# muzishen/IMAGHarmony

Hardware: AMD Instinct MI355X
Metric: 1024^2 SDXL images/sec (30 DDIM steps, PNS N seeds) (higher is better)
Workload: dtype bf16

## Files before the change

### imagharmony_amd/csrc/api.hip

```cpp
#include <stdarg.h>
#include <stdio.h>
#include <string.h>

#include <vector>

#include "../../include/imh.h"
#include "../../include/imh_adapter.h"
#include "../../include/imh_regions.h"
#include "imh_common.h"
#include "imh_kernels.h"

namespace imh {

static thread_local char g_err[512] = "";

void set_error(const char* fmt, ...) {
    va_list ap;
    va_start(ap, fmt);
    vsnprintf(g_err, sizeof(g_err), fmt, ap);
    va_end(ap);
}

int experimental_refused(const char* what) {
    set_error("%s is compiled only with -DIMH_EXPERIMENTAL (IMH_EXPERIMENTAL=1 python -m imagharmony_amd.build): measured, not selected by any "
// ... 275 lines not shown
    p.mean[0] = a->mean0; p.mean[1] = a->mean1; p.mean[2] = a->mean2; p.std[0] = a->std0; p.std[1] = a->std1; p.std[2] = a->std2;
    p.ncols = p.ntx = p.nty = p.RC = 0;
    return clip_preprocess_launch(p, a->dtype, s);
}

static int do_control_add(const imh_control_add_args* a, hipStream_t s) {
    const char* who = "imh_control_add";
    if (!a || !a->x || !a->r || !a->y) { set_error("%s: null pointer argument", who); return IMH_ERR_ARG; }
    if (((uintptr_t)a->x | (uintptr_t)a->r | (uintptr_t)a->y) & 15) { set_error("%s: x, r and y must be 16-byte aligned", who); return IMH_ERR_ARG; }
    if (((uintptr_t)a->partial | (uintptr_t)a->tab | (uintptr_t)a->step) & 3) { set_error("%s: partial, tab and step must be 4-byte aligned", who); return IMH_ERR_ARG; }
    if ((a->tab == nullptr) != (a->step == nullptr)) { set_error("%s: tab and step come together", who); return IMH_ERR_ARG; }
    if (a->B <= 0 || a->HW <= 0 || a->C <= 0 || a->Br <= 0) { set_error("%s: B=%d Br=%d HW=%d C=%d must be positive", who, a->B, a->Br, a->HW, a->C); return IMH_ERR_SHAPE; }
    const size_t yb = (size_t)a->B * a->HW * a->C * 2, rb = (size_t)a->Br * a->HW * a->C * 2;
    const uintptr_t y0 = (uintptr_t)a->y, x0 = (uintptr_t)a->x, r0 = (uintptr_t)a->r;
    if ((y0 < x0 + yb && x0 < y0 + yb) || (y0 < r0 + rb && r0 < y0 + yb)) { set_error("%s: y must not overlap x or r (no in-place form)", who); return IMH_ERR_ARG; }
    ControlAddParams p;
    p.x = a->x; p.r = a->r; p.y = a->y; p.partial = a->partial; p.tab = a->tab; p.step = a->step; p.scale = a->scale;
    p.B = a->B; p.Br = a->Br; p.HW = a->HW; p.C = a->C; p.sub = a->sub;
    return control_add_launch(p, a->dtype, s);
}

static int do_adapter_op(const imh_adapter_args* a, hipStream_t s) {
    const char* who = "imh_adapter_op";
    if (!a || !a->x || !a->y) { set_error("%s: null pointer argument", who); return IMH_ERR_ARG; }
    if (a->mode != IMH_ADAPTER_UNSHUFFLE && a->mode != IMH_ADAPTER_RELU && a->mode != IMH_ADAPTER_AVGPOOL2) {
        set_error("%s: unknown mode %d", who, a->mode); return IMH_ERR_ARG;
    }
    if (((uintptr_t)a->y & 15) || ((uintptr_t)a->x & (a->mode == IMH_ADAPTER_UNSHUFFLE ? 3 : 15))) {
        set_error("%s: y (and x, unshuffle: to 4 bytes) must be 16-byte aligned", who); return IMH_ERR_ARG;
    }
    if (a->dtype != IMH_DT_BF16 && a->dtype != IMH_DT_F16) { set_error("%s: unknown dtype %d", who, a->dtype); return IMH_ERR_DTYPE; }
    const long long lim = 0x7fffffffLL;
    long long xe, ye;
    if (a->mode == IMH_ADAPTER_RELU) {
        if (a->n <= 0 || a->n > lim) { set_error("%s: relu over n=%lld elements (0 < n < 2^31)", who, (long long)a->n); return IMH_ERR_SHAPE; }
        xe = ye = a->n;
    } else {
        if (a->N <= 0 || a->C <= 0 || a->H <= 0 || a->W <= 0) { set_error("%s: N=%d C=%d H=%d W=%d must be positive", who, a->N, a->C, a->H, a->W); return IMH_ERR_SHAPE; }
        xe = (long long)a->N * a->C;
        if (xe > lim || (xe *= a->H) > lim || (xe *= a->W) > lim) { set_error("%s: N=%d C=%d H=%d W=%d: an operand of 2^31 elements or more", who, a->N, a->C, a->H, a->W); return IMH_ERR_SHAPE; }
        if (a->mode == IMH_ADAPTER_UNSHUFFLE) {
            if (a->f < 1 || a->H % a->f || a->W % a->f) { set_error("%s: unshuffle of %d x %d by f=%d (f >= 1 divides both sides)", who, a->H, a->W, a->f); return IMH_ERR_SHAPE; }
            const long long K = (long long)a->C * a->f * a->f;
            if (a->Cp <= 0 || a->Cp % 8 || a->Cp < K) { set_error("%s: Cp=%d must be a multiple of 8 and at least C f^2 = %lld", who, a->Cp, K); return IMH_ERR_SHAPE; }
            ye = (long long)a->N * (a->H / a->f) * (a->W / a->f);
            if (ye > lim || (ye *= a->Cp) > lim) { set_error("%s: Cp=%d: an operand of 2^31 elements or more", who, a->Cp); return IMH_ERR_SHAPE; }
        } else {
            if (a->C % 8) { set_error("%s: avgpool2 over C=%d channels (a multiple of 8)", who, a->C); return IMH_ERR_SHAPE; }
            ye = (long long)a->N * ((a->H + 1) / 2) * ((a->W + 1) / 2) * a->C;
        }
    }
    const uintptr_t x0 = (uintptr_t)a->x, y0 = (uintptr_t)a->y;
    const size_t xb = (size_t)xe * (a->mode == IMH_ADAPTER_UNSHUFFLE ? 4 : 2), yb = (size_t)ye * 2;
    if (y0 < x0 + xb && x0 < y0 + yb && !(a->mode == IMH_ADAPTER_RELU && x0 == y0)) {
        set_error("%s: y must not overlap x (relu: except y == x)", who); return IMH_ERR_ARG;
    }
    AdapterParams p;
    p.x = a->x; p.y = a->y; p.n = a->n; p.mode = a->mode; p.N = a->N; p.C = a->C; p.H = a->H; p.W = a->W; p.f = a->f; p.Cp = a->Cp;
    return adapter_launch(p, a->dtype, s);
}

}

using namespace imh;

struct imh_op {
    int kind;
    int ew_op;
    int tag;
    union {
        imh_gemm_args gemm;
        imh_attn_args attn;
        imh_norm_args norm;
        imh_ew_args ew;
        imh_small_attn_args sattn;
        imh_gemm_args gemm2[2];
        imh_xattn_args xattn;
        imh_enc_attn_args eattn;
        imh_seeded_args seeded;
        imh_randn_args randn;
        imh_clip_preprocess_args clip;
        imh_control_add_args cadd;
        imh_xattn_regions_args xregions;
    } u;
};

struct imh_plan {
    std::vector<imh_op> ops;
    hipGraph_t graph = nullptr;
    hipGraphExec_t exec = nullptr;
};

struct op_entry {
    int kind;
    size_t size;
    int (*run)(const imh_op&, hipStream_t);
};
static const op_entry g_ops[] = {
    {IMH_OP_GEMM, sizeof(imh_gemm_args), [](const imh_op& o, hipStream_t s) { return do_gemm(&o.u.gemm, s); }},
    {IMH_OP_ATTN, sizeof(imh_attn_args), [](const imh_op& o, hipStream_t s) { return do_attn(&o.u.attn, s); }},
    {IMH_OP_GROUPNORM, sizeof(imh_norm_args), [](const imh_op& o, hipStream_t s) { return do_groupnorm(&o.u.norm, s); }},
    {IMH_OP_LAYERNORM, sizeof(imh_norm_args), [](const imh_op& o, hipStream_t s) { return do_layernorm(&o.u.norm, s); }},
    {IMH_OP_EW, sizeof(imh_ew_args), [](const imh_op& o, hipStream_t s) { return do_ew(o.ew_op, &o.u.ew, s); }},
    {IMH_OP_ATTN_SMALL, sizeof(imh_small_attn_args), [](const imh_op& o, hipStream_t s) { return do_attn_small(&o.u.sattn, s); }},
    {IMH_OP_GEMM_DUAL, 2 * sizeof(imh_gemm_args), [](const imh_op& o, hipStream_t s) { return do_gemm_dual(&o.u.gemm2[0], &o.u.gemm2[1], s); }},
    {IMH_OP_XATTN, sizeof(imh_xattn_args), [](const imh_op& o, hipStream_t s) { return do_xattn(&o.u.xattn, s); }},
    {IMH_OP_ATTN_ENC, sizeof(imh_enc_attn_args), [](const imh_op& o, hipStream_t s) { return do_attn_enc(&o.u.eattn, s); }},
    {IMH_OP_ATTN_ENC_CAUSAL, sizeof(imh_enc_attn_args), [](const imh_op& o, hipStream_t s) { return do_attn_enc(&o.u.eattn, s, 1); }},
    {IMH_OP_STEP_SEEDED, sizeof(imh_seeded_args), [](const imh_op& o, hipStream_t s) { return do_step_seeded(&o.u.seeded, s); }},
    {IMH_OP_RANDN_SEEDED, sizeof(imh_randn_args), [](const imh_op& o, hipStream_t s) { return do_randn_seeded(&o.u.randn, s); }},
    {IMH_OP_CLIP_PREPROCESS, sizeof(imh_clip_preprocess_args), [](const imh_op& o, hipStream_t s) { return do_clip_preprocess(&o.u.clip, s); }},
    {IMH_OP_CONTROL_ADD, sizeof(imh_control_add_args), [](const imh_op& o, hipStream_t s) { return do_control_add(&o.u.cadd, s); }},
    {IMH_OP_XATTN_REGIONS, sizeof(imh_xattn_regions_args), [](const imh_op& o, hipStream_t s) { return do_xattn_regions(&o.u.xregions, s); }},
};

static const op_entry* find_op(int kind) {
    for (const op_entry& e : g_ops)
        if (e.kind == kind) return &e;
    return nullptr;
}

static int run_op(const imh_op& o, hipStream_t s) {
    const op_entry* e = find_op(o.kind);
    if (!e) { set_error("plan: unknown op kind %d", o.kind); return IMH_ERR_ARG; }
    return e->run(o, s);
}

static void drop_graph(imh_plan* p) {
    if (p->exec) { hipGraphExecDestroy(p->exec); p->exec = nullptr; }
    if (p->graph) { hipGraphDestroy(p->graph); p->graph = nullptr; }
}

extern "C" {

int imh_abi_version(void) { return IMH_ABI_VERSION; }
int imh_debug_set(int key, int value) {
    if (key == 0) { g_attn_force_nw = value; return IMH_OK; }
    if (key == 1) {
#ifdef IMH_EXPERIMENTAL
        return 1;
#else
        return 0;
#endif
    }
    if (key == 2) { g_xcd_mode = value; return IMH_OK; }
    if (key == 3) { g_xattn_mode = value; return IMH_OK; }
    if (key == 4) { g_attn_mode = value; return IMH_OK; }
    if (key == 5) { g_halo_mode = value; return IMH_OK; }
    if (key == 7) { g_w16_pf = value; return IMH_OK; }
    if (key == 9) { g_w16_form = value; return IMH_OK; }
    if (key == 10) { g_f32_exact = value; return IMH_OK; }
    if (key == 11) { if (value >= 0) g_up_phase = value; return g_up_phase; }
    if (key == 6) { g_ws_early = value; return IMH_OK; }
    set_error("debug_set: unknown key %d", key);
    return IMH_ERR_ARG;
}
const char* imh_last_error(void) { return g_err; }

int imh_gemm(const imh_gemm_args* a, void* stream) { return do_gemm(a, (hipStream_t)stream); }
int imh_gemm_dual(const imh_gemm_args* a, const imh_gemm_args* b, void* stream) { return do_gemm_dual(a, b, (hipStream_t)stream); }
int imh_gemm_pick_config(int M, int N, int K, int* bm, int* bn, int* splits) {
    if (!bm || !bn || !splits) { set_error("pick_config: null output"); return IMH_ERR_ARG; }
    gemm_pick_config(M, N, K, bm, bn, splits);
    return IMH_OK;
}
size_t imh_gemm_workspace_bytes(int M, int N, int splits) { return gemm_workspace_bytes(M, N, splits); }
int imh_gemm_stats_slot_width(int bm, int bn) { return gemm_stats_slot_width(bm, bn); }
int imh_gemm_gn_block_rows(int bm, int bn) { return gemm_gn_block_rows(bm, bn); }
int imh_conv_halo_lds_bytes(int bm, int bn, int Cin, int gn) { return conv_halo_lds_bytes(bm, bn, Cin, gn); }

int imh_gemm_check(const imh_gemm_args* a) {
    static thread_local std::vector<hipStream_t> streams;
    int dev = -1;
    if (hipGetDevice(&dev) != hipSuccess || dev < 0) { (void)hipGetLastError(); set_error("gemm_check: no current device"); return IMH_ERR_LAUNCH; }
    if ((size_t)dev >= streams.size()) streams.resize(dev + 1, nullptr);
    hipStream_t& cs = streams[dev];
    if (!cs && hipStreamCreateWithFlags(&cs, hipStreamNonBlocking) != hipSuccess) {
        cs = nullptr; (void)hipGetLastError();
        set_error("gemm_check: no stream to validate on"); return IMH_ERR_LAUNCH;
    }
    hipError_t e = hipStreamBeginCapture(cs, hipStreamCaptureModeThreadLocal);
    if (e != hipSuccess) { (void)hipGetLastError(); set_error("gemm_check: begin: %s", hipGetErrorString(e)); return IMH_ERR_LAUNCH; }
    const int rc = do_gemm(a, cs);
    hipGraph_t g = nullptr;
    e = hipStreamEndCapture(cs, &g);
    if (g) hipGraphDestroy(g);
    if (rc != IMH_OK) { (void)hipGetLastError(); return rc; }
    if (e != hipSuccess) { (void)hipGetLastError(); set_error("gemm_check: end: %s", hipGetErrorString(e)); return IMH_ERR_LAUNCH; }
    return IMH_OK;
}

int imh_attention(const imh_attn_args* a, void* stream) { return do_attn(a, (hipStream_t)stream); }

int imh_cross_attention(const imh_xattn_args* a, void* stream) { return do_xattn(a, (hipStream_t)stream); }

int imh_cross_attention_regions(const imh_xattn_regions_args* a, void* stream) { return do_xattn_regions(a, (hipStream_t)stream); }

int imh_attention_small(const imh_small_attn_args* a, void* stream) { return do_attn_small(a, (hipStream_t)stream); }

int imh_attention_enc(const imh_enc_attn_args* a, void* stream) { return do_attn_enc(a, (hipStream_t)stream); }
int imh_attention_enc_causal(const imh_enc_attn_args* a, void* stream) { return do_attn_enc(a, (hipStream_t)stream, 1); }

int imh_groupnorm(const imh_norm_args* a, void* stream) { return do_groupnorm(a, (hipStream_t)stream); }
size_t imh_groupnorm_workspace_bytes(int B, int HW, int C, int groups) { return groupnorm_workspace_bytes(B, HW, C, groups); }
int imh_groupnorm_stats_blocks(int HW, int C) { return groupnorm_stats_blocks(HW, C); }
int imh_groupnorm_stats_sub(int C, int groups) { return groups > 0 && C % groups == 0 ? groupnorm_stats_sub(C, groups) : 0; }
int imh_layernorm(const imh_norm_args* a, void* stream) { return do_layernorm(a, (hipStream_t)stream); }

int imh_elementwise(int op, const imh_ew_args* a, void* stream) { return do_ew(op, a, (hipStream_t)stream); }

int imh_step_seeded(const imh_seeded_args* a, void* stream) { return do_step_seeded(a, (hipStream_t)stream); }
int imh_randn_seeded(const imh_randn_args* a, void* stream) { return do_randn_seeded(a, (hipStream_t)stream); }
int imh_clip_preprocess(const imh_clip_preprocess_args* a, void* stream) { return do_clip_preprocess(a, (hipStream_t)stream); }
int imh_control_add(const imh_control_add_args* a, void* stream) { return do_control_add(a, (hipStream_t)stream); }
int imh_adapter_op(const imh_adapter_args* a, void* stream) { return do_adapter_op(a, (hipStream_t)stream); }
int imh_randn_seeded_host(const imh_randn_args* a) {
    RandnParams p;
    const int rc = to_randn(a, "imh_randn_seeded_host", &p);
    return rc != IMH_OK ? rc : randn_seeded_host(p);
}

int imh_f32(int op, const imh_f32_args* a, void* stream) {
    if (!a) { set_error("imh_f32: null args"); return IMH_ERR_ARG; }
    F32Params p;
    p.X = a->X; p.W = a->W; p.Y = a->Y; p.bias = a->bias; p.residual = a->residual; p.gamma = a->gamma; p.beta = a->beta; p.ws = a->ws;
    p.M = a->M; p.N = a->N; p.K = a->K; p.ldx = a->ldx; p.ldw = a->ldw; p.ldy = a->ldy; p.ldr = a->ldr;
    p.conv = a->conv; p.H = a->H; p.Wd = a->Wd; p.Cin = a->Cin; p.Ho = a->Ho; p.Wo = a->Wo; p.up = a->up;
    p.B = a->B; p.HW = a->HW; p.C = a->C; p.groups = a->groups; p.nblk = a->nblk; p.silu = a->silu;
    p.eps = a->eps; p.scale = a->scale;
    if (a->pad != 0 && a->pad != 1) { set_error("imh_f32: pad must be 0 or 1"); return IMH_ERR_ARG; }
    p.stride = a->stride > 0 ? a->stride : 1; p.pad_lo = a->pad == 1 ? 0 : 1;
    p.add_a = a->add_a; p.add_b = a->add_b;
    return f32_launch(op, p, (hipStream_t)stream);
}

imh_plan* imh_plan_create(void) { return new (std::nothrow) imh_plan(); }
void imh_plan_destroy(imh_plan* p) {
    if (!p) return;
    drop_graph(p);
    delete p;
}
int imh_plan_add(imh_plan* p, int kind, const void* args, int ew_op, int tag) {
    if (!p || !args) { set_error("plan_add: null argument"); return IMH_ERR_ARG; }
    const op_entry* e = find_op(kind);
    if (!e) { set_error("plan_add: unknown kind %d", kind); return IMH_ERR_ARG; }
    imh_op o;
    memset(&o, 0, sizeof(o));
    o.kind = kind; o.ew_op = ew_op; o.tag = tag;
    memcpy(&o.u, args, e->size);
    p->ops.push_back(o);
    drop_graph(p);
    return (int)p->ops.size() - 1;
}
int imh_plan_size(const imh_plan* p) { return p ? (int)p->ops.size() : 0; }
int imh_plan_update(imh_plan* p, int index, const void* args) {
    if (!p || !args || index < 0 || index >= (int)p->ops.size()) { set_error("plan_update: bad index"); return IMH_ERR_ARG; }
    memcpy(&p->ops[index].u, args, find_op(p->ops[index].kind)->size);
    drop_graph(p);
    return IMH_OK;
}
int imh_plan_run_range(imh_plan* p, int first, int last, void* stream) {
    if (!p || first < 0 || last > (int)p->ops.size() || first > last) { set_error("plan_run: bad range"); return IMH_ERR_ARG; }
    for (int i = first; i < last; ++i) {
        int rc = run_op(p->ops[i], (hipStream_t)stream);
        if (rc != IMH_OK) return rc;
    }
    return IMH_OK;
}
int imh_plan_run(imh_plan* p, void* stream) { return imh_plan_run_range(p, 0, p ? (int)p->ops.size() : 0, stream); }

int imh_plan_capture(imh_plan* p, void* stream) {
    if (!p) { set_error("plan_capture: null plan"); return IMH_ERR_ARG; }
    drop_graph(p);
    hipStream_t s = (hipStream_t)stream;
    hipError_t e = hipStreamBeginCapture(s, hipStreamCaptureModeThreadLocal);
    if (e != hipSuccess) { set_error("plan_capture: begin: %s", hipGetErrorString(e)); return IMH_ERR_LAUNCH; }
    int rc = imh_plan_run(p, stream);
    e = hipStreamEndCapture(s, &p->graph);
    if (rc != IMH_OK) { drop_graph(p); return rc; }
    if (e != hipSuccess) { set_error("plan_capture: end: %s", hipGetErrorString(e)); drop_graph(p); return IMH_ERR_LAUNCH; }
    e = hipGraphInstantiate(&p->exec, p->graph, nullptr, nullptr, 0);
    if (e != hipSuccess) { set_error("plan_capture: instantiate: %s", hipGetErrorString(e)); drop_graph(p); return IMH_ERR_LAUNCH; }
    return IMH_OK;
}
int imh_plan_replay(imh_plan* p, void* stream) {
    if (!p || !p->exec) { set_error("plan_replay: plan not captured"); return IMH_ERR_ARG; }
    hipError_t e = hipGraphLaunch(p->exec, (hipStream_t)stream);
    if (e != hipSuccess) { set_error("plan_replay: %s", hipGetErrorString(e)); return IMH_ERR_LAUNCH; }
    return IMH_OK;
}
int imh_plan_time_ops(imh_plan* p, void* stream, float* ms, int n) {
    if (!p || !ms || n < (int)p->ops.size()) { set_error("plan_time_ops: bad arguments"); return IMH_ERR_ARG; }
    hipStream_t s = (hipStream_t)stream;
    const int cnt = (int)p->ops.size();
    std::vector<hipEvent_t> ev(cnt + 1);
    for (auto& e : ev) hipEventCreate(&e);
    int rc = IMH_OK;
    hipEventRecord(ev[0], s);
    for (int i = 0; i < cnt && rc == IMH_OK; ++i) {
        rc = run_op(p->ops[i], s);
        hipEventRecord(ev[i + 1], s);
    }
    hipStreamSynchronize(s);
    if (rc == IMH_OK)
        for (int i = 0; i < cnt; ++i) hipEventElapsedTime(&ms[i], ev[i], ev[i + 1]);
    for (auto& e : ev) hipEventDestroy(e);
// ... 11 lines not shown
```

### imagharmony_amd/csrc/elementwise.hip

```cpp
#include <algorithm>

#include "imh_common.h"
#include "imh_kernels.h"
#include "imh_philox.h"

namespace imh {

enum : int { EW_TIMESTEP = 0, EW_SILU = 1, EW_CONCAT = 2, EW_CONV_IN = 3, EW_CFG_STEP = 4, EW_CAST_F32 = 5,
             EW_ADD = 6, EW_STEP_SET = 7, EW_CFG_RESCALE = 8, EW_SOFTMAX = 9, EW_ROW_STATS = 10, EW_STEP_ROW = 11, EW_GATHER_ROWS = 12,
             EW_CFG_MSTEP = 13 };

template <typename T>
__global__ void timestep_kernel(const EwParams p) {
    const int dim = p.i0, half = dim >> 1;
    const long long total = p.n * half;
    for (long long i = (long long)blockIdx.x * blockDim.x + threadIdx.x; i < total; i += (long long)gridDim.x * blockDim.x) {
        const int v = (int)(i / half), j = (int)(i % half);
        const float t = p.step ? ((const float*)p.a)[*p.step] : ((const float*)p.a)[v];
        const float f = expf(-9.210340371976184f * (float)j / (float)half);
        const float a = t * f;
        T* y = (T*)p.y + (size_t)v * dim;
        y[j] = from_f32<T>(cosf(a));
        y[half + j] = from_f32<T>(sinf(a));
    }
}

template <typename T>
__global__ void silu_kernel(const EwParams p) {
    typedef typename Vec<T>::v8 v8;
    const long long nv = p.n >> 3;
    for (long long i = (long long)blockIdx.x * blockDim.x + threadIdx.x; i < nv; i += (long long)gridDim.x * blockDim.x) {
        v8 v = ((const v8*)p.a)[i], o;
#pragma unroll
        for (int e = 0; e < 8; ++e) o[e] = from_f32<T>(silu_f(to_f32(v[e])));
        ((v8*)p.y)[i] = o;
    }
}

template <typename T>
__global__ void add_kernel(const EwParams p) {
    typedef typename Vec<T>::v8 v8;
    const long long nv = p.n >> 3;
    for (long long i = (long long)blockIdx.x * blockDim.x + threadIdx.x; i < nv; i += (long long)gridDim.x * blockDim.x) {
        v8 u = ((const v8*)p.a)[i], v = ((const v8*)p.b)[i], o;
#pragma unroll
        for (int e = 0; e < 8; ++e) o[e] = from_f32<T>(to_f32(u[e]) + to_f32(v[e]));
        ((v8*)p.y)[i] = o;
    }
}

template <typename T>
__global__ void concat_kernel(const EwParams p) {
    typedef typename Vec<T>::v8 v8;
    const int c1 = p.i0 >> 3, c2 = p.i1 >> 3, ct = c1 + c2;
    const long long total = p.n * ct;
    for (long long i = (long long)blockIdx.x * blockDim.x + threadIdx.x; i < total; i += (long long)gridDim.x * blockDim.x) {
        const long long pix = i / ct;
        const int c = (int)(i - pix * ct);
        v8 v = c < c1 ? ((const v8*)p.a)[pix * c1 + c] : ((const v8*)p.b)[pix * c2 + (c - c1)];
        ((v8*)p.y)[i] = v;
    }
}

template <typename T, int CIN>
__global__ __launch_bounds__(CIN > 4 ? 512 : 256) void conv_in_kernel(const EwParams p) {
    typedef typename Vec<T>::v8 v8;
    constexpr int KT = CIN * 9;
    extern __shared__ float wl[];
    const int S = p.i0, H = p.i1, W = p.i2, C0 = p.i3, Bout = p.i4;
    const T* w = (const T*)p.w;
    for (int co = threadIdx.x; co < C0; co += blockDim.x) {
#pragma unroll
        for (int k = 0; k < KT; ++k) wl[k * C0 + co] = to_f32(w[co * KT + k]);
    }
    for (int i = threadIdx.x; i < C0; i += blockDim.x) wl[KT * C0 + i] = p.bias ? to_f32(((const T*)p.bias)[i]) : 0.f;
    __syncthreads();
    const int cg = C0 >> 3;
    const float in_scale = p.tab ? p.tab[*p.step] : p.f0;
    const long long total = (long long)Bout * H * W * 8;
    const float* lat = (const float*)p.a;
    for (long long i = (long long)blockIdx.x * blockDim.x + threadIdx.x; i < total; i += (long long)gridDim.x * blockDim.x) {
        const int l8 = (int)(i & 7);
        const long long pix = i >> 3;
        const int x = (int)(pix % W);
        const int y = (int)((pix / W) % H);
        const int b = (int)(pix / ((long long)W * H));
        const float* src = lat + (size_t)(b % S) * 4 * H * W;
        float tap[KT];
#pragma unroll
        for (int ci = 0; ci < 4; ++ci)
#pragma unroll
            for (int ky = 0; ky < 3; ++ky)
#pragma unroll
                for (int kx = 0; kx < 3; ++kx) {
                    const int iy = y + ky - 1, ix = x + kx - 1;
                    const bool in = iy >= 0 && iy < H && ix >= 0 && ix < W;
                    const float v = in ? src[((size_t)ci * H + iy) * W + ix] * in_scale : 0.f;
                    tap[ci * 9 + ky * 3 + kx] = to_f32(from_f32<T>(v));
                }
        if constexpr (CIN > 4) {
            const float* src2 = p.x2 + (size_t)(b % S) * (CIN - 4) * H * W;
#pragma unroll
            for (int ci = 4; ci < CIN; ++ci)
#pragma unroll
                for (int ky = 0; ky < 3; ++ky)
#pragma unroll
                    for (int kx = 0; kx < 3; ++kx) {
                        const int iy = y + ky - 1, ix = x + kx - 1;
                        const bool in = iy >= 0 && iy < H && ix >= 0 && ix < W;
                        const float v = in ? src2[((size_t)(ci - 4) * H + iy) * W + ix] : 0.f;
                        tap[ci * 9 + ky * 3 + kx] = to_f32(from_f32<T>(v));
                    }
        }
        for (int c8 = l8; c8 < cg; c8 += 8) {
            float acc[8];
#pragma unroll
            for (int e = 0; e < 8; ++e) acc[e] = wl[KT * C0 + c8 * 8 + e];
#pragma unroll
            for (int k = 0; k < KT; ++k) {
                const float* wr = wl + k * C0 + c8 * 8;
#pragma unroll
                for (int e = 0; e < 8; ++e) acc[e] += tap[k] * wr[e];
            }
            v8 o;
#pragma unroll
            for (int e = 0; e < 8; ++e) o[e] = from_f32<T>(acc[e]);
            ((v8*)p.y)[pix * cg + c8] = o;
        }
    }
}

template <typename T, bool BLEND>
__global__ void cfg_step_kernel(const EwParams p) {
    const int S = p.i0, HW = p.i1;
    const long long total = (long long)S * HW * 4;
    const T* np_ = (const T*)p.a;
    float* lat = (float*)p.y;
    const float cx = p.tab ? p.tab[*p.step * 2] : p.f0;
    const float ce = p.tab ? p.tab[*p.step * 2 + 1] : p.f1;
    float ba = 0.f, bb = 0.f;
    if constexpr (BLEND) { ba = p.blend_tab[*p.step * 2]; bb = p.blend_tab[*p.step * 2 + 1]; }
    for (long long i = (long long)blockIdx.x * blockDim.x + threadIdx.x; i < total; i += (long long)gridDim.x * blockDim.x) {
        const int pix = (int)(i % HW);
        const int ch = (int)((i / HW) % 4);
        const int s = (int)(i / ((long long)HW * 4));
        if (!BLEND || np_) {
            float eps;
            if (p.i3) {
                const float u = to_f32(np_[((size_t)s * HW + pix) * 4 + ch]);
                const float c = to_f32(np_[((size_t)(S + s) * HW + pix) * 4 + ch]);
                eps = u + p.f2 * (c - u);
            } else {
                eps = to_f32(np_[((size_t)s * HW + pix) * 4 + ch]);
            }
            if (p.w) eps *= ((const float*)p.w)[s];
            if (p.b) ((float*)p.b)[i] = eps;
            lat[i] = cx * lat[i] + ce * eps;
        }
        if constexpr (BLEND) {
            const float m = p.mask[(size_t)(s % p.i4) * HW + pix];
            const float pv = ba * p.x2[i] + bb * p.noise[i];
            lat[i] = (1.0f - m) * pv + m * lat[i];
        }
    }
}

template <typename T, bool BLEND, bool SEEDED = false>
__global__ void cfg_mstep_kernel(const EwParams p) {
    const int S = p.i0, HW = p.i1;
    const long long total = (long long)S * HW * 4;
    const T* np_ = (const T*)p.a;
    float* lat = (float*)p.y;
    float* hist = (float*)p.b;
    const int row = *p.step;
    const float* c = p.tab + (size_t)row * 6;
    const float cx = c[0], ce = c[1], ch = c[2], cn = c[3], hx = c[4], he = c[5];
    const float* z = p.bias ? (const float*)p.bias + (size_t)row * (size_t)total : nullptr;
    float ba = 0.f, bb = 0.f;
    if constexpr (BLEND) { ba = p.blend_tab[row * 2]; bb = p.blend_tab[row * 2 + 1]; }
    if constexpr (SEEDED) {
        const bool gen = cn != 0.f;
        const long long quads = (long long)S * HW;
        for (long long q = (long long)blockIdx.x * blockDim.x + threadIdx.x; q < quads; q += (long long)gridDim.x * blockDim.x) {
            const int s = (int)(q / HW);
            PhiloxNormals zn = {{0.f, 0.f, 0.f, 0.f}};
            if (gen) zn = seeded_normals(p.seeds + (size_t)s * 4, (uint32_t)(q - (long long)s * HW), (uint32_t)row, p.noise_stream);
#pragma unroll
            for (int k = 0; k < 4; ++k) {
                const long long i = q * 4 + k;
                const int pix = (int)(i % HW);
                const int chn = (int)((i / HW) % 4);
                float eps;
                if (p.i3) {
                    const float u = to_f32(np_[((size_t)s * HW + pix) * 4 + chn]);
                    const float cnd = to_f32(np_[((size_t)(S + s) * HW + pix) * 4 + chn]);
                    eps = u + p.f2 * (cnd - u);
                } else {
                    eps = to_f32(np_[((size_t)s * HW + pix) * 4 + chn]);
                }
                if (p.w) eps *= ((const float*)p.w)[s];
                const float x = lat[i];
                float y = cx * x + ce * eps;
                if (hist) {
                    y += ch * hist[i];
                    hist[i] = hx * x + he * eps;
                }
                if (gen) y += cn * zn.z[k];
                if constexpr (BLEND) {
                    const float m = p.mask[(size_t)(s % p.i4) * HW + pix];
                    const float pv = ba * p.x2[i] + bb * p.noise[i];
                    y = (1.0f - m) * pv + m * y;
                }
                lat[i] = y;
            }
        }
        return;
    }
    for (long long i = (long long)blockIdx.x * blockDim.x + threadIdx.x; i < total; i += (long long)gridDim.x * blockDim.x) {
        const int pix = (int)(i % HW);
        const int chn = (int)((i / HW) % 4);
        const int s = (int)(i / ((long long)HW * 4));
        float eps;
        if (p.i3) {
            const float u = to_f32(np_[((size_t)s * HW + pix) * 4 + chn]);
            const float cnd = to_f32(np_[((size_t)(S + s) * HW + pix) * 4 + chn]);
            eps = u + p.f2 * (cnd - u);
        } else {
            eps = to_f32(np_[((size_t)s * HW + pix) * 4 + chn]);
        }
        if (p.w) eps *= ((const float*)p.w)[s];
        const float x = lat[i];
        float y = cx * x + ce * eps;
        if (hist) {
            y += ch * hist[i];
            hist[i] = hx * x + he * eps;
        }
        if (z) y += cn * z[i];
        if constexpr (BLEND) {
            const float m = p.mask[(size_t)(s % p.i4) * HW + pix];
            const float pv = ba * p.x2[i] + bb * p.noise[i];
            y = (1.0f - m) * pv + m * y;
        }
        lat[i] = y;
    }
}

__global__ void randn_seeded_kernel(const RandnParams p) {
    const int HW = p.HW;
    const uint32_t row = p.step ? (uint32_t)*p.step : p.row;
    const long long quads = (long long)p.S * HW;
    for (long long q = (long long)blockIdx.x * blockDim.x + threadIdx.x; q < quads; q += (long long)gridDim.x * blockDim.x) {
        const int s = (int)(q / HW);
        const uint32_t qs = p.quad0 + (uint32_t)(q - (long long)s * HW);
        if (p.raw) {
            const PhiloxWords w = seeded_words(p.seeds + (size_t)s * 4, qs, row, p.noise_stream);
            uint32_t* y = (uint32_t*)p.y + q * 4;
#pragma unroll
            for (int k = 0; k < 4; ++k) y[k] = w.w[k];
        } else {
            const PhiloxNormals n = seeded_normals(p.seeds + (size_t)s * 4, qs, row, p.noise_stream);
            float* y = (float*)p.y + q * 4;
#pragma unroll
            for (int k = 0; k < 4; ++k) y[k] = n.z[k];
        }
    }
}

template <typename T>
__global__ __launch_bounds__(256) void cfg_rescale_kernel(const EwParams p) {
    __shared__ double red[4][256];
    const int S = p.i0, HW = p.i1, s = blockIdx.x;
    const long long n = (long long)HW * 4;
    const T* u = (const T*)p.a + (size_t)s * n;
    const T* c = (const T*)p.a + (size_t)(S + s) * n;
    double st = 0, st2 = 0, sc = 0, sc2 = 0;
    for (long long i = threadIdx.x; i < n; i += 256) {
        const float uu = to_f32(u[i]), cc = to_f32(c[i]);
        const float g = uu + p.f2 * (cc - uu);
        st += cc; st2 += (double)cc * cc; sc += g; sc2 += (double)g * g;
    }
    red[0][threadIdx.x] = st; red[1][threadIdx.x] = st2; red[2][threadIdx.x] = sc; red[3][threadIdx.x] = sc2;
// ... 1 lines not shown
    for (int o = 128; o > 0; o >>= 1) {
        if ((int)threadIdx.x < o)
#pragma unroll
            for (int k = 0; k < 4; ++k) red[k][threadIdx.x] += red[k][threadIdx.x + o];
        __syncthreads();
    }
    if (threadIdx.x == 0) {
        const double N = (double)n;
        const double vt = (red[1][0] - red[0][0] * red[0][0] / N) / (N - 1.0);
        const double vc = (red[3][0] - red[2][0] * red[2][0] / N) / (N - 1.0);
        const double ratio = sqrt(fmax(vt, 0.0)) / sqrt(fmax(vc, 1e-300));
        ((float*)p.y)[s] = (float)(p.f3 * ratio + (1.0 - p.f3));
    }
}

template <typename T>
__global__ __launch_bounds__(256) void softmax_rows_kernel(const EwParams p) {
    __shared__ float red[4];
    const int cols = p.i1, lane = threadIdx.x & 63, wave = threadIdx.x >> 6;
    const float* a = (const float*)p.a + (size_t)blockIdx.x * p.i2;
    T* y = (T*)p.y + (size_t)blockIdx.x * p.i3;
    const float c = p.f0 * 1.4426950408889634f;
    float m = -3.0e38f;
    for (int i = threadIdx.x * 4; i < cols; i += 1024) {
        const f32x4 v = *(const f32x4*)(a + i);
        m = fmaxf(fmaxf(m, fmaxf(v[0], v[1])), fmaxf(v[2], v[3]));
    }
    m = wave_max(m);
    if (lane == 0) red[wave] = m;
    __syncthreads();
    m = fmaxf(fmaxf(red[0], red[1]), fmaxf(red[2], red[3]));
    __syncthreads();
    const float mc = m * c;
    float s = 0.f;
    for (int i = threadIdx.x * 4; i < cols; i += 1024) {
        const f32x4 v = *(const f32x4*)(a + i);
#pragma unroll
        for (int e = 0; e < 4; ++e) s += __builtin_amdgcn_exp2f(v[e] * c - mc);
    }
    s = wave_sum(s);
    if (lane == 0) red[wave] = s;
    __syncthreads();
    const float inv = 1.0f / ((red[0] + red[1]) + (red[2] + red[3]));
    for (int i = threadIdx.x * 4; i < cols; i += 1024) {
        const f32x4 v = *(const f32x4*)(a + i);
        typename Vec<T>::v4 o;
#pragma unroll
        for (int e = 0; e < 4; ++e) o[e] = from_f32<T>(__builtin_amdgcn_exp2f(v[e] * c - mc) * inv);
        *(typename Vec<T>::v4*)(y + i) = o;
    }
}

template <typename T>
__global__ void step_row_kernel(const EwParams p) {
    typedef typename Vec<T>::v8 v8;
    const long long nv = p.n >> 3;
    const v8* src = (const v8*)p.a + (long long)(*p.step) * nv;
    for (long long i = (long long)blockIdx.x * blockDim.x + threadIdx.x; i < nv; i += (long long)gridDim.x * blockDim.x) ((v8*)p.y)[i] = src[i];
}

template <typename T>
__global__ void gather_rows_kernel(const EwParams p) {
    typedef typename Vec<T>::v8 v8;
    const int cv = p.i0 >> 3;
    const long long total = p.n * cv;
    const int* idx = (const int*)p.b;
    for (long long i = (long long)blockIdx.x * blockDim.x + threadIdx.x; i < total; i += (long long)gridDim.x * blockDim.x) {
        const long long r = i / cv;
        const int c = (int)(i - r * cv) * 8;
        const int src = idx[r];
        if ((unsigned)src >= (unsigned)p.i5) continue;
        v8 v = *(const v8*)((const T*)p.a + (size_t)src * p.i1 + c);
        if (p.w) {
            const v8 u = *(const v8*)((const T*)p.w + (size_t)(r % p.i3) * p.i4 + c);
#pragma unroll
            for (int e = 0; e < 8; ++e) v[e] = from_f32<T>(to_f32(v[e]) + to_f32(u[e]));
        }
        *(v8*)((T*)p.y + (size_t)r * p.i2 + c) = v;
    }
}

__global__ void step_set_kernel(int* step, int value, int set) {
    if (threadIdx.x == 0 && blockIdx.x == 0) *step = set ? value : *step + 1;
}

template <typename T>
__global__ void cast_f32_kernel(const EwParams p) {
    for (long long i = (long long)blockIdx.x * blockDim.x + threadIdx.x; i < p.n; i += (long long)gridDim.x * blockDim.x)
        ((float*)p.y)[i] = to_f32(((const T*)p.a)[i]);
}

static inline int grid_for(long long work, int threads) {
    long long g = (work + threads - 1) / threads;
    return (int)(g < 1 ? 1 : (g > 4096 ? 4096 : g));
}

template <typename T>
__global__ __launch_bounds__(256) void row_stats_kernel(const EwParams p) {
    const int lane = threadIdx.x & 63;
    const long long row = (long long)blockIdx.x * 4 + (threadIdx.x >> 6);
    if (row >= p.n) return;
    const T* x = (const T*)p.a + row * p.i1;
    const int C = p.i0;
    float s = 0.f;
    for (int c = lane * 8; c < C; c += 512) {
        const typename Vec<T>::v8 t = *(const typename Vec<T>::v8*)(x + c);
#pragma unroll
        for (int e = 0; e < 8; ++e) s += to_f32(t[e]);
    }
    s = wave_sum(s);
    const float mean = s / (float)C;
    float m2 = 0.f;
    for (int c = lane * 8; c < C; c += 512) {
        const typename Vec<T>::v8 t = *(const typename Vec<T>::v8*)(x + c);
#pragma unroll
        for (int e = 0; e < 8; ++e) { const float d = to_f32(t[e]) - mean; m2 = __builtin_fmaf(d, d, m2); }
    }
    m2 = wave_sum(m2);
    if (lane == 0) { float* y = (float*)p.y + row * 2; y[0] = s; y[1] = m2; }
}

template <typename T>
static int ew_typed(int op, const EwParams& p, hipStream_t stream) {
    switch (op) {
        case EW_TIMESTEP:
            if (p.i0 <= 0 || (p.i0 & 1)) { set_error("timestep: dim must be even"); return IMH_ERR_SHAPE; }
            hipLaunchKernelGGL((timestep_kernel<T>), dim3(grid_for(p.n * (p.i0 >> 1), 256)), dim3(256), 0, stream, p);
            break;
        case EW_SILU:
            if (p.n & 7) { set_error("silu: n must be a multiple of 8"); return IMH_ERR_SHAPE; }
            hipLaunchKernelGGL((silu_kernel<T>), dim3(grid_for(p.n >> 3, 256)), dim3(256), 0, stream, p);
            break;
        case EW_ADD:
            if (p.n & 7) { set_error("add: n must be a multiple of 8"); return IMH_ERR_SHAPE; }
            hipLaunchKernelGGL((add_kernel<T>), dim3(grid_for(p.n >> 3, 256)), dim3(256), 0, stream, p);
            break;
        case EW_CONCAT:
            if ((p.i0 & 7) || (p.i1 & 7)) { set_error("concat: channel counts must be multiples of 8"); return IMH_ERR_SHAPE; }
            hipLaunchKernelGGL((concat_kernel<T>), dim3(grid_for(p.n * ((p.i0 + p.i1) >> 3), 256)), dim3(256), 0, stream, p);
            break;
        case EW_CONV_IN: {
            if (p.i3 & 7) { set_error("conv_in: C0 must be a multiple of 8"); return IMH_ERR_SHAPE; }
            const long long work = (long long)p.i4 * p.i1 * p.i2 * 8;
            if (p.i5 == 9) {
                static DynLdsOnce once;
                const size_t lds = (size_t)(82 * p.i3) * sizeof(float);
                if (!p.x2 || p.i0 <= 0) { set_error("conv_in: 9 input channels need the second source x2 [S, 5, H, W]"); return IMH_ERR_ARG; }
                if (lds > 160 * 1024) { set_error("conv_in: C0 = %d needs %zu bytes of LDS at 9 input channels (160 KiB per workgroup)", p.i3, lds); return IMH_ERR_SHAPE; }
                if (lds > 64 * 1024) once.ensure((const void*)conv_in_kernel<T, 9>, 160 * 1024);
                hipLaunchKernelGGL((conv_in_kernel<T, 9>), dim3(std::min(grid_for(work, 512), lds > 53 * 1024 ? 256 : 768)), dim3(512), lds, stream, p);
                break;
            }
            if (p.i5 != 0 && p.i5 != 4) { set_error("conv_in: %d input channels (4 or 9)", p.i5); return IMH_ERR_ARG; }
            const size_t lds = (size_t)(37 * p.i3) * sizeof(float);
            hipLaunchKernelGGL((conv_in_kernel<T, 4>), dim3(std::min(grid_for(work, 256), 768)), dim3(256), lds, stream, p);
            break;
        }
        case EW_CFG_STEP:
            if (p.mask) {
                if (!p.x2 || !p.noise || !p.blend_tab || !p.step || p.i4 < 1) {
                    set_error("cfg_step: the masked blend needs x2 (image latents), noise, blend_tab, step and i4 = mask batch >= 1");
                    return IMH_ERR_ARG;
                }
                hipLaunchKernelGGL((cfg_step_kernel<T, true>), dim3(grid_for((long long)p.i0 * p.i1 * 4, 256)), dim3(256), 0, stream, p);
                break;
            }
            if (!p.a) { set_error("cfg_step: null noise prediction"); return IMH_ERR_ARG; }
            hipLaunchKernelGGL((cfg_step_kernel<T, false>), dim3(grid_for((long long)p.i0 * p.i1 * 4, 256)), dim3(256), 0, stream, p);
            break;
        case EW_CFG_MSTEP:
            if (!p.a || !p.tab || !p.step || p.i0 <= 0 || p.i1 <= 0) {
                set_error("cfg_mstep: needs the noise prediction, the six-column table, step and S, HW > 0");
                return IMH_ERR_ARG;
            }
            if (p.mask) {
                if (!p.x2 || !p.noise || !p.blend_tab || p.i4 < 1) {
                    set_error("cfg_mstep: the masked blend needs x2 (image latents), noise, blend_tab and i4 = mask batch >= 1");
                    return IMH_ERR_ARG;
                }
                if (p.seeds) hipLaunchKernelGGL((cfg_mstep_kernel<T, true, true>), dim3(grid_for((long long)p.i0 * p.i1, 256)), dim3(256), 0, stream, p);
                else hipLaunchKernelGGL((cfg_mstep_kernel<T, true>), dim3(grid_for((long long)p.i0 * p.i1 * 4, 256)), dim3(256), 0, stream, p);
                break;
            }
            if (p.seeds) hipLaunchKernelGGL((cfg_mstep_kernel<T, false, true>), dim3(grid_for((long long)p.i0 * p.i1, 256)), dim3(256), 0, stream, p);
            else hipLaunchKernelGGL((cfg_mstep_kernel<T, false>), dim3(grid_for((long long)p.i0 * p.i1 * 4, 256)), dim3(256), 0, stream, p);
            break;
        case EW_CFG_RESCALE:
            if (p.i0 <= 0 || p.i1 <= 0) { set_error("cfg_rescale: empty problem"); return IMH_ERR_SHAPE; }
            hipLaunchKernelGGL((cfg_rescale_kernel<T>), dim3(p.i0), dim3(256), 0, stream, p);
            break;
        case EW_SOFTMAX:
            if (p.i0 <= 0 || p.i1 <= 0 || (p.i1 & 3) || (p.i2 & 3) || (p.i3 & 3) || p.f0 <= 0.f) {
                set_error("softmax: rows=%d cols=%d ld=%d/%d (cols and lds must be multiples of 4, scale > 0)", p.i0, p.i1, p.i2, p.i3);
                return IMH_ERR_SHAPE;
            }
            hipLaunchKernelGGL((softmax_rows_kernel<T>), dim3(p.i0), dim3(256), 0, stream, p);
            break;
        case EW_CAST_F32:
            hipLaunchKernelGGL((cast_f32_kernel<T>), dim3(grid_for(p.n, 256)), dim3(256), 0, stream, p);
            break;
        case EW_ROW_STATS:
            if (p.n <= 0 || p.i0 <= 0 || (p.i0 & 7) || (p.i1 & 7) || !p.a) { set_error("row_stats: rows=%lld C=%d ld=%d (C and ld must be multiples of 8)", p.n, p.i0, p.i1); return IMH_ERR_SHAPE; }
            hipLaunchKernelGGL((row_stats_kernel<T>), dim3((unsigned)((p.n + 3) / 4)), dim3(256), 0, stream, p);
            break;
        case EW_STEP_ROW:
            if (p.n <= 0 || (p.n & 7) || !p.a || !p.step) { set_error("step_row: n=%lld must be a positive multiple of 8, a and step non-null", p.n); return IMH_ERR_ARG; }
            hipLaunchKernelGGL((step_row_kernel<T>), dim3(grid_for(p.n >> 3, 256)), dim3(256), 0, stream, p);
            break;
        case EW_GATHER_ROWS:
            if (!p.a || !p.b || p.n <= 0 || p.i0 <= 0 || (p.i0 & 7) || p.i1 < p.i0 || (p.i1 & 7) || p.i2 < p.i0 || (p.i2 & 7) || p.i5 <= 0 ||
                (p.w && (p.i3 <= 0 || p.i4 < p.i0 || (p.i4 & 7)))) {
                set_error("gather_rows: n=%lld C=%d ld=%d/%d table rows=%d add rows=%d ld=%d (table, idx non-null; C and the row strides multiples of 8, "
                          "strides >= C; table rows > 0; with add: rows > 0)", p.n, p.i0, p.i1, p.i2, p.i5, p.i3, p.i4);
                return IMH_ERR_SHAPE;
            }
            if ((((uintptr_t)p.a | (uintptr_t)p.y | (uintptr_t)p.w) & 15) || ((uintptr_t)p.b & 3)) {
                set_error("gather_rows: table / add / y must be 16-byte aligned, idx 4-byte aligned"); return IMH_ERR_ARG;
            }
            hipLaunchKernelGGL((gather_rows_kernel<T>), dim3(grid_for(p.n * (p.i0 >> 3), 256)), dim3(256), 0, stream, p);
            break;
        case EW_STEP_SET:
            hipLaunchKernelGGL(step_set_kernel, dim3(1), dim3(64), 0, stream, (int*)p.y, p.i0, p.i1);
            break;
        default:
            set_error("elementwise: unknown op %d", op);
            return IMH_ERR_ARG;
    }
    return check_launch("elementwise");
}

int randn_seeded_launch(const RandnParams& p, hipStream_t stream) {
    hipLaunchKernelGGL(randn_seeded_kernel, dim3(grid_for((long long)p.S * p.HW, 256)), dim3(256), 0, stream, p);
    return check_launch("randn_seeded");
}

int randn_seeded_host(const RandnParams& p) {
    const uint32_t row = p.step ? (uint32_t)*p.step : p.row;
    for (int s = 0; s < p.S; ++s)
        for (int q = 0; q < p.HW; ++q) {
            const size_t o = ((size_t)s * p.HW + q) * 4;
            if (p.raw) {
                const PhiloxWords w = seeded_words(p.seeds + (size_t)s * 4, p.quad0 + (uint32_t)q, row, p.noise_stream);
                for (int k = 0; k < 4; ++k) ((uint32_t*)p.y)[o + k] = w.w[k];
            } else {
                const PhiloxNormals n = seeded_normals(p.seeds + (size_t)s * 4, p.quad0 + (uint32_t)q, row, p.noise_stream);
                for (int k = 0; k < 4; ++k) ((float*)p.y)[o + k] = n.z[k];
            }
        }
    return IMH_OK;
}

int ew_launch(int op, const EwParams& p, int dtype, hipStream_t stream) {
    if (dtype == IMH_DT_BF16) return ew_typed<bf16_t>(op, p, stream);
    if (dtype == IMH_DT_F16) return ew_typed<f16_t>(op, p, stream);
    set_error("elementwise: unknown dtype %d", dtype);
    return IMH_ERR_DTYPE;
}

}
```

### imagharmony_amd/csrc/imh_kernels.h

```cpp
#pragma once
#include <hip/hip_runtime.h>
#include <stddef.h>
#include "imh_gntable.h"

namespace imh {

struct GemmParams {
    const void* X;
    const void* W;
    void* Y;
    float* partial;
    const void* bias;
    const void* rowadd;
    const void* residual;
    const float* ln_s;
    const float* ln_c;
    float ln_eps;
    const float* ln_stats;
    float* ln_stats_out;
    int ln_slots, ln_slots_out;
    float* gn_out;
    int gn_nblk, gn_hw;
    const float* gn_tab;
    int gn_silu;
    GnTabSrc gn_src;
    const void* X2;
    int Cin1;
    void* Yt;
    int yt_col0, ldyt;
    int M, N, K;
    int ldx, ldw, ldy, ldr, ldra;
    int rows_per_batch;
    int splits;
    int flags;
    int H, Wd, Cin, Ho, Wo, stride, up, pad_lo;
    int phase, pN;
    int px, py, tmx, tny;
    int xcd;
    const void* pf_ptr;
    unsigned pf_bytes;
    int early_res;
};

inline bool variant_is_ws(int bm) { return bm == 1464 || bm == 2464 || bm == 24128 || bm == 23256 || bm == 22128; }
inline bool variant_is_halo(int bm) { return bm >= 7000 && bm < 8000; }

void gemm_pick_config(int M, int N, int K, int* bm, int* bn, int* splits);
size_t gemm_workspace_bytes(int M, int N, int splits);
int gemm_stats_slot_width(int bm, int bn);
int gemm_gn_block_rows(int bm, int bn);
int gemm_launch(GemmParams p, int dtype, int conv, int bm, int bn, hipStream_t stream);
int gemm_dual_launch(GemmParams a, GemmParams b, int dtype, int bm, int bn, hipStream_t stream);
int gemm_w16_launch(const GemmParams& p, int dtype, hipStream_t stream);
int conv_halo_lds_bytes(int bm, int bn, int Cin, int gn);

struct AttnParams {
    const void* Q;
    const void* K;
    const void* Vt;
    const void* K2;
    const void* Vt2;
    void* O;
    int B, H, Lq;
    int Lk, Lk_pad;
    int Lk2, Lk2_pad;
    int ldq, ldk, ldvt, ldk2, ldvt2, ldo;
    float scale;
    float scale2;
    const float* scale2_tab;
    const int* step;
    const void* pf_ptr;
    unsigned pf_bytes;
    int split;
    float defer_log2;
};
int attention_launch(const AttnParams& p, int dtype, hipStream_t stream);

struct XAttnParams {
    AttnParams a;
    const void* X;
    const void* Wq;
    const float* ln_s;
    const float* ln_c;
    float ln_eps;
    const float* ln_stats;
    int ln_slots;
    int C, ldx, ldw;
    int split;
};
int xattn_launch(const XAttnParams& p, int dtype, hipStream_t stream);

constexpr int XR_MAX_IMAGES = 8;
struct XRegionParams {
    XAttnParams x;
    const float* mask;
    const float* weights;
    int n_img, ldm;
};
int xattn_regions_launch(const XRegionParams& p, int dtype, hipStream_t stream);
extern int g_attn_force_nw;
extern int g_xattn_mode;
extern int g_w16_pf;
extern int g_w16_form;
extern int g_f32_exact;
extern int g_attn_mode;
extern int g_xcd_mode;
extern int g_halo_mode;
extern int g_ws_early;
extern int g_up_phase;

struct SmallAttnParams {
    const void* Q; const void* K; const void* V; void* O;
    int B, H, Lq, Lk, dq, dv;
    int ldq, ldk, ldv, ldo;
    float scale;
};
int attention_small_launch(const SmallAttnParams& p, int dtype, hipStream_t stream);

struct EncAttnParams {
    const void* Q; const void* K; const void* V; void* O;
    int B, H, L, d;
    int ldq, ldk, ldv, ldo;
    float scale;
    int causal;
};
int attention_enc_launch(const EncAttnParams& p, int dtype, hipStream_t stream);

struct NormParams {
    const void* x;
    void* y;
    const void* gamma;
    const void* beta;
    float* partial;
    int B, HW, C, groups;
    int rows;
    float eps;
    int silu;
    int mode;
    float* table;
    const float* partial2;
    int nblk, sub, npart;
    int C1;
    int nblk2, sub2, npart2;
    int dtype_f16;
    const void* pf_ptr;
    unsigned pf_bytes;
};
int groupnorm_launch(const NormParams& p, int dtype, hipStream_t stream);
size_t groupnorm_workspace_bytes(int B, int HW, int C, int groups);
int groupnorm_stats_blocks(int HW, int C);
int groupnorm_stats_sub(int C, int groups);
int layernorm_launch(const NormParams& p, int dtype, hipStream_t stream);

struct ControlAddParams {
    const void* x; const void* r; void* y;
    float* partial;
    const float* tab; const int* step;
    float scale;
    int B, Br, HW, C, sub;
};
int control_add_launch(const ControlAddParams& p, int dtype, hipStream_t stream);

struct AdapterParams {
    const void* x; void* y;
    long long n;
    int mode, N, C, H, W, f, Cp;
};
int adapter_launch(const AdapterParams& p, int dtype, hipStream_t stream);

struct F32Params {
    const float* X; const float* W; float* Y; const float* bias; const float* residual; const float* gamma; const float* beta; float* ws;
    int M, N, K, ldx, ldw, ldy, ldr;
    int conv, H, Wd, Cin, Ho, Wo, up;
    int B, HW, C, groups, nblk, silu;
    float eps, scale;
    int stride, pad_lo;
    float add_a, add_b;
};
int f32_launch(int op, const F32Params& p, hipStream_t stream);

struct EwParams {
    const void* a;
    const void* b;
    void* y;
    const void* w;
    const void* bias;
    const float* tab;
    const int* step;
    long long n;
    int i0, i1, i2, i3, i4, i5;
    float f0, f1, f2, f3;
    const float* x2;
    const float* noise;
    const float* mask;
    const float* blend_tab;
    const unsigned* seeds = nullptr;
    unsigned noise_stream = 0;
};
int ew_launch(int op, const EwParams& p, int dtype, hipStream_t stream);

struct RandnParams {
    void* y;
    const unsigned* seeds;
    const int* step;
    int S, HW;
    unsigned row, noise_stream;
    int raw;
    unsigned quad0;
};
int randn_seeded_launch(const RandnParams& p, hipStream_t stream);
int randn_seeded_host(const RandnParams& p);

struct ClipPreParams {
    const float* x;
    void* y;
    int S, H, W;
    int nh, nw, top, left;
    int size, patch, ldp;
    float mean[3], std[3];
    int ncols, ntx, nty, RC;
};
int clip_preprocess_launch(ClipPreParams p, int dtype, hipStream_t stream);

}
```

Before: 1.765.

## Add tiled conv_in kernel with spatial patch and output-channel-group tiling

Adds a new conv_in kernel for 4-channel latents. Each workgroup stages one spatial patch of the input and the weights for a group of 64 output channels in LDS, and each thread computes 4 adjacent pixels times 8 channels from a register sliding window. Batch-duplicated outputs are written from the same accumulators. This is meant to cut redundant weight and input reloads compared with the old per-pixel grid-stride kernel. A debug flag can restore the old path; the gain is small because conv_in is a tiny share of the SDXL step.

Result: no change. 1.765 (-0.0%).

```diff
diff --git a/imagharmony_amd/csrc/api.hip b/imagharmony_amd/csrc/api.hip
--- a/imagharmony_amd/csrc/api.hip
+++ b/imagharmony_amd/csrc/api.hip
@@ -451,6 +451,7 @@
     if (key == 10) { g_f32_exact = value; return IMH_OK; }
     if (key == 11) { if (value >= 0) g_up_phase = value; return g_up_phase; }
     if (key == 6) { g_ws_early = value; return IMH_OK; }
+    if (key == 12) { if (value >= 0) g_small_old = value; return g_small_old; }
     set_error("debug_set: unknown key %d", key);
     return IMH_ERR_ARG;
 }
diff --git a/imagharmony_amd/csrc/elementwise.hip b/imagharmony_amd/csrc/elementwise.hip
--- a/imagharmony_amd/csrc/elementwise.hip
+++ b/imagharmony_amd/csrc/elementwise.hip
@@ -3,8 +3,11 @@
 #include "imh_common.h"
 #include "imh_kernels.h"
 #include "imh_philox.h"
+#include "imh_small_index.h"
 
 namespace imh {
+
+int g_small_old = 0;
 
 enum : int { EW_TIMESTEP = 0, EW_SILU = 1, EW_CONCAT = 2, EW_CONV_IN = 3, EW_CFG_STEP = 4, EW_CAST_F32 = 5,
              EW_ADD = 6, EW_STEP_SET = 7, EW_CFG_RESCALE = 8, EW_SOFTMAX = 9, EW_ROW_STATS = 10, EW_STEP_ROW = 11, EW_GATHER_ROWS = 12,
@@ -127,6 +130,77 @@
             for (int e = 0; e < 8; ++e) o[e] = from_f32<T>(acc[e]);
             ((v8*)p.y)[pix * cg + c8] = o;
         }
+    }
+}
+
+template <typename T>
+IMH_KERNEL __launch_bounds__(CI_THREADS, 4) void conv_in_tile_kernel(const EwParams p) {
+    typedef typename Vec<T>::v8 v8;
+    constexpr int GC = CI_OG * 8;
+    __shared__ __attribute__((aligned(16))) float wl[37 * GC];
+    __shared__ float pt[CI_PATCH];
+    const int S = p.i0, H = p.i1, W = p.i2, C0 = p.i3, Bout = p.i4;
+    const ConvInGrid g = conv_in_grid(S, Bout, H, W, C0);
+    const ConvInItem it = conv_in_item(g, blockIdx.x);
+    const int t = threadIdx.x;
+    const int nch = conv_in_group_channels(it.og, C0);
+    {
+        const v8* w8 = (const v8*)((const T*)p.w + (size_t)it.og * GC * 36);
+        for (int i = t; i < nch * 36 / 8; i += CI_THREADS) {
+            const v8 v = w8[i];
+#pragma unroll
+            for (int e = 0; e < 8; ++e) {
+                const int f = i * 8 + e, co = f / 36;
+                wl[(f - co * 36) * GC + co] = to_f32(v[e]);
+            }
+        }
+        if (t < GC) wl[36 * GC + t] = (p.bias && t < nch) ? to_f32(((const T*)p.bias)[it.og * GC + t]) : 0.f;
+    }
+    const float in_scale = p.tab ? p.tab[*p.step] : p.f0;
+    const float* src = (const float*)p.a + (size_t)it.b * 4 * H * W;
+    for (int i = t; i < CI_PATCH; i += CI_THREADS) {
+        const long long o = conv_in_patch_src(it, i, H, W);
+        const float v = o >= 0 ? src[o] * in_scale : 0.f;
+        pt[i] = to_f32(from_f32<T>(v));
+    }
+    __builtin_amdgcn_fence(__ATOMIC_RELEASE, "workgroup");
+    __builtin_amdgcn_s_barrier();
+    __builtin_amdgcn_fence(__ATOMIC_ACQUIRE, "workgroup");
+    int y, x0, oc;
+    if (!conv_in_thread(it, t, H, W, C0, y, x0, oc)) return;
+    float acc[CI_QW][8];
+    const float* wb = wl + (t & 7) * 8;
+#pragma unroll
+    for (int j = 0; j < CI_QW; ++j)
+#pragma unroll
+        for (int e = 0; e < 8; ++e) acc[j][e] = wb[36 * GC + e];
+#pragma unroll 1
+    for (int ci = 0; ci < 4; ++ci) {
+        float win[3][CI_QW + 2];
+#pragma unroll
+        for (int ky = 0; ky < 3; ++ky)
+#pragma unroll
+            for (int m = 0; m < CI_QW + 2; ++m) win[ky][m] = pt[conv_in_patch_at(t, ci, ky, m)];
+#pragma unroll
+        for (int ky = 0; ky < 3; ++ky)
+#pragma unroll
+            for (int kx = 0; kx < 3; ++kx) {
+                const float* wr = wb + (ci * 9 + ky * 3 + kx) * GC;
+#pragma unroll
+                for (int j = 0; j < CI_QW; ++j) {
+                    const float tap = win[ky][j + kx];
+#pragma unroll
+                    for (int e = 0; e < 8; ++e) acc[j][e] += tap * wr[e];
+                }
+            }
+    }
+#pragma unroll
+    for (int j = 0; j < CI_QW; ++j) {
+        if (x0 + j >= W) break;
+        v8 o;
+#pragma unroll
+        for (int e = 0; e < 8; ++e) o[e] = from_f32<T>(acc[j][e]);
+        for (int bb = it.b; bb < Bout; bb += S) ((v8*)p.y)[conv_in_out_octet(bb, y, x0 + j, oc, H, W, C0)] = o;
     }
 }
 
@@ -434,6 +508,13 @@
                 break;
             }
             if (p.i5 != 0 && p.i5 != 4) { set_error("conv_in: %d input channels (4 or 9)", p.i5); return IMH_ERR_ARG; }
+            if (!(g_small_old & 1) && !((uintptr_t)p.w & 15) && p.i0 > 0 && p.i4 > 0 && p.i1 > 0 && p.i2 > 0 && p.i3 > 0) {
+                const long long nwg = conv_in_workgroups(conv_in_grid(p.i0, p.i4, p.i1, p.i2, p.i3));
+                if (nwg <= 0x7fffffffLL) {
+                    hipLaunchKernelGGL((conv_in_tile_kernel<T>), dim3((unsigned)nwg), dim3(CI_THREADS), 0, stream, p);
+                    break;
+                }
+            }
             const size_t lds = (size_t)(37 * p.i3) * sizeof(float);
             hipLaunchKernelGGL((conv_in_kernel<T, 4>), dim3(std::min(grid_for(work, 256), 768)), dim3(256), lds, stream, p);
             break;
diff --git a/imagharmony_amd/csrc/imh_kernels.h b/imagharmony_amd/csrc/imh_kernels.h
--- a/imagharmony_amd/csrc/imh_kernels.h
+++ b/imagharmony_amd/csrc/imh_kernels.h
@@ -108,6 +108,7 @@
 extern int g_halo_mode;
 extern int g_ws_early;
 extern int g_up_phase;
+extern int g_small_old;
 
 struct SmallAttnParams {
     const void* Q; const void* K; const void* V; void* O;
diff --git a/imagharmony_amd/csrc/imh_small_index.h b/imagharmony_amd/csrc/imh_small_index.h
--- /dev/null
+++ b/imagharmony_amd/csrc/imh_small_index.h
@@ -0,0 +1,67 @@
+#pragma once
+
+#if defined(__HIPCC__)
+#define IMH_SK_HD __host__ __device__ __forceinline__
+#else
+#define IMH_SK_HD inline
+#endif
+
+namespace imh {
+
+constexpr int CI_THREADS = 256;
+constexpr int CI_TW = 32, CI_TH = 4;
+constexpr int CI_QW = 4;
+constexpr int CI_OG = 8;
+constexpr int CI_PW = CI_TW + 2, CI_PH = CI_TH + 2;
+constexpr int CI_PATCH = 4 * CI_PH * CI_PW;
+static_assert(CI_THREADS == (CI_TW / CI_QW) * CI_TH * CI_OG, "one thread per (quad, octet of the group)");
+
+struct ConvInGrid {
+    int nb, nty, ntx, nog;
+};
+IMH_SK_HD ConvInGrid conv_in_grid(int S, int Bout, int H, int W, int C0) {
+    ConvInGrid g;
+    g.nb = S < Bout ? S : Bout;
+    g.nty = (H + CI_TH - 1) / CI_TH;
+    g.ntx = (W + CI_TW - 1) / CI_TW;
+    g.nog = ((C0 >> 3) + CI_OG - 1) / CI_OG;
+    return g;
+}
+IMH_SK_HD long long conv_in_workgroups(const ConvInGrid& g) { return (long long)g.nb * g.nty * g.ntx * g.nog; }
+
+struct ConvInItem { int b, ty, tx, og; };
+IMH_SK_HD ConvInItem conv_in_item(const ConvInGrid& g, long long wg) {
+    ConvInItem it;
+    it.og = (int)(wg % g.nog); wg /= g.nog;
+    it.tx = (int)(wg % g.ntx); wg /= g.ntx;
+    it.ty = (int)(wg % g.nty);
+    it.b = (int)(wg / g.nty);
+    return it;
+}
+
+IMH_SK_HD bool conv_in_thread(const ConvInItem& it, int t, int H, int W, int C0, int& y, int& x0, int& oc) {
+    const int q = t >> 3;
+    y = it.ty * CI_TH + q / (CI_TW / CI_QW);
+    x0 = it.tx * CI_TW + (q % (CI_TW / CI_QW)) * CI_QW;
+    oc = it.og * CI_OG + (t & 7);
+    return y < H && x0 < W && oc < (C0 >> 3);
+}
+IMH_SK_HD int conv_in_patch_at(int t, int ci, int ky, int m) {
+    const int q = t >> 3;
+    return (ci * CI_PH + q / (CI_TW / CI_QW) + ky) * CI_PW + (q % (CI_TW / CI_QW)) * CI_QW + m;
+}
+IMH_SK_HD long long conv_in_patch_src(const ConvInItem& it, int i, int H, int W) {
+    const int c = i % CI_PW, r = (i / CI_PW) % CI_PH, ci = i / (CI_PW * CI_PH);
+    const int iy = it.ty * CI_TH + r - 1, ix = it.tx * CI_TW + c - 1;
+    if (iy < 0 || iy >= H || ix < 0 || ix >= W) return -1;
+    return ((long long)ci * H + iy) * W + ix;
+}
+IMH_SK_HD int conv_in_group_channels(int og, int C0) {
+    const int n = C0 - og * CI_OG * 8;
+    return n < CI_OG * 8 ? n : CI_OG * 8;
+}
+IMH_SK_HD long long conv_in_out_octet(int bb, int y, int x, int oc, int H, int W, int C0) {
+    return (((long long)bb * H + y) * W + x) * (C0 >> 3) + oc;
+}
+
+}
```
